# codgodtao/TMDiff

Hardware: AMD Instinct MI355X
Metric: UNet denoise-steps/sec (8-ch 64x64, batch 32) (higher is better)
Workload: dtype f32; 1 GPU; BASELINE configs[1]: batch-32 8-ch 64x64 tiles, DDPM p_sample steps of the T=1000 cosine schedule, channel_multiplier [32,64,128,256], full UNet forward (both branches) + fused DDPM update per step; batch_per_gpu=32, parallelism=batch-parallel x1, weights=key-hashed random init, text_embedding=fixed synthetic 768-d

## Files before the change

include/tmdiff_hip.h:

```cpp
#ifndef TMDIFF_HIP_H
#define TMDIFF_HIP_H

#include <stddef.h>
#include <stdint.h>

#ifdef __cplusplus
extern "C" {
#endif

#define TMDIFF_ABI_VERSION 6

#define TMDIFF_OK 0
#define TMDIFF_E_INVALID (-1)
#define TMDIFF_E_UNSUPPORTED (-2)
#define TMDIFF_E_LAUNCH (-3)

typedef void* tmdiff_stream_t;

int tmdiff_version(void);
const char* tmdiff_last_error_string(void);

typedef struct tmdiff_conv3d_desc {
  int32_t B, N, H, W;
  int32_t Cin, Cout;
// ... 71 lines not shown
int tmdiff_conv3d_wino_pack_weights(const float* w, float* packed, int32_t Cout, int32_t Cin, int32_t groups,
                                    int32_t mode, int32_t planes, tmdiff_stream_t stream);
typedef struct tmdiff_wino_pack_entry {
  const float* w;
  float* packed;
  int32_t Cout, Cin, groups, mode, planes, reserved;
} tmdiff_wino_pack_entry;
int32_t tmdiff_conv3d_wino_pack_weights_multi_chunk(void);
int tmdiff_conv3d_wino_pack_weights_multi(const tmdiff_wino_pack_entry* entries_dev, const int32_t* chunk_tensor_dev,
                                          const int32_t* chunk_index_dev, int32_t n_chunks, tmdiff_stream_t stream);
int tmdiff_conv3d_wino_fwd(const tmdiff_conv3d_desc* d, void* workspace, tmdiff_stream_t stream);
int tmdiff_conv3d_wino_fwd_stage(const tmdiff_conv3d_desc* d, void* workspace, int32_t stage, tmdiff_stream_t stream);
int tmdiff_conv3d_wino_fwd_xp(const tmdiff_conv3d_desc* d, void* workspace, int32_t stage, float* xp_out, tmdiff_stream_t stream);
int tmdiff_conv3d_wino_fwd_planes(const tmdiff_conv3d_desc* d, void* workspace, int32_t stage, float* xp_out, int32_t planes,
                                  tmdiff_stream_t stream);

int tmdiff_conv3d_wf_supported(const tmdiff_conv3d_desc* d);
int64_t tmdiff_conv3d_wf_blocks(const tmdiff_conv3d_desc* d);
size_t tmdiff_conv3d_wf_splitk_workspace_bytes(const tmdiff_conv3d_desc* d);
size_t tmdiff_conv3d_wf_workspace_bytes(const tmdiff_conv3d_desc* d);
int32_t tmdiff_conv3d_wf_plan(int32_t B, int32_t Cin, int32_t Cout, int32_t N, int32_t H, int32_t W, int32_t groups, int32_t llm,
                              int64_t* tiles);
int tmdiff_conv3d_wf_fwd(const tmdiff_conv3d_desc* d, void* workspace, tmdiff_stream_t stream);
int tmdiff_conv3d_wfll_supported(const tmdiff_conv3d_desc* d);
size_t tmdiff_conv3d_wfll_packed_bytes(int32_t Cout, int32_t Cin);
int tmdiff_conv3d_wfll_pack_weights(const float* w, float* packed, int32_t Cout, int32_t Cin, float ll_scale,
                                    tmdiff_stream_t stream);
size_t tmdiff_conv3d_wfll_splitk_workspace_bytes(const tmdiff_conv3d_desc* d);
int tmdiff_conv3d_wfll_fwd(const tmdiff_conv3d_desc* d, float ll_scale, tmdiff_stream_t stream);

size_t tmdiff_conv3d_packed_bf16_bytes(int32_t Cout, int32_t Cin, int32_t ksize, int32_t groups);
int tmdiff_conv3d_pack_weights_bf16(const float* w, void* packed, int32_t Cout, int32_t Cin, int32_t ksize,
                                    int32_t groups, tmdiff_stream_t stream);
int tmdiff_conv3d_pack_weights_bf16_dgrad(const float* w, void* packed, int32_t Cout, int32_t Cin, int32_t ksize,
                                          int32_t groups, tmdiff_stream_t stream);
size_t tmdiff_conv3d_bf16_workspace_bytes(const tmdiff_conv3d_desc* d);
int tmdiff_conv3d_fwd_bf16(const tmdiff_conv3d_desc* d, void* workspace, tmdiff_stream_t stream);


int tmdiff_conv3d_prologue_fwd(const tmdiff_conv3d_desc* d, float* xp, tmdiff_stream_t stream);

size_t tmdiff_conv3d_wgrad_workspace_bytes(const tmdiff_conv3d_desc* d);
int tmdiff_conv3d_wgrad(const tmdiff_conv3d_desc* d, const float* g, float* dw, void* workspace,
                        tmdiff_stream_t stream);
int tmdiff_conv3d_wgrad_bias(const tmdiff_conv3d_desc* d, const float* g, float* dw, float* dbias, void* workspace,
                             tmdiff_stream_t stream);
// ... 261 lines not shown
```

tmdiff_amd/_lib.py:

```python
import ctypes as C
import os

_HERE = os.path.dirname(os.path.abspath(__file__))
LIB_PATH = os.environ.get("TMDIFF_HIP_LIB") or os.path.join(_HERE, "libtmdiff_hip.so")

c_float_p = C.POINTER(C.c_float)
vp = C.c_void_p


class Conv3dDesc(C.Structure):
    _fields_ = [
        ("B", C.c_int32), ("N", C.c_int32), ("H", C.c_int32), ("W", C.c_int32),
        ("Cin", C.c_int32), ("Cout", C.c_int32),
        ("groups", C.c_int32), ("ksize", C.c_int32), ("nseg", C.c_int32),
        ("seg_c", C.c_int32 * 3),
        ("seg_x", vp * 3),
        ("w_packed", vp), ("bias", vp), ("bias_scale", C.c_float),
        ("in_shift", vp), ("in_scale", vp), ("in_shift_stride", C.c_int32), ("in_scale_stride", C.c_int32),
        ("in_mask", vp), ("in_act", C.c_int32),
        ("residual", vp), ("out_scale", C.c_float),
        ("y", vp),
        ("y2", vp), ("y2_shift", vp), ("y2_scale", vp), ("y2_shift_stride", C.c_int32), ("y2_scale_stride", C.c_int32),
        ("y2_act", C.c_int32), ("y2_bf16", C.c_int32), ("x_bf16", C.c_int32),
        ("splitk_ws", vp), ("splitk_ws_bytes", C.c_int64),
# ... 25 lines not shown
    "tmdiff_conv3d_wf_supported": (C.c_int, [C.POINTER(Conv3dDesc)]),
    "tmdiff_conv3d_wf_blocks": (C.c_int64, [C.POINTER(Conv3dDesc)]),
    "tmdiff_conv3d_wf_workspace_bytes": (C.c_size_t, [C.POINTER(Conv3dDesc)]),
    "tmdiff_conv3d_wf_splitk_workspace_bytes": (C.c_size_t, [C.POINTER(Conv3dDesc)]),
    "tmdiff_conv3d_wf_fwd": (C.c_int, [C.POINTER(Conv3dDesc), vp, vp]),
    "tmdiff_conv3d_wino_fwd": (C.c_int, [C.POINTER(Conv3dDesc), vp, vp]),
    "tmdiff_conv3d_wino_fwd_planes": (C.c_int, [C.POINTER(Conv3dDesc), vp, C.c_int32, vp, C.c_int32, vp]),
    "tmdiff_conv3d_wino_fwd_xp": (C.c_int, [C.POINTER(Conv3dDesc), vp, C.c_int32, vp, vp]),
    "tmdiff_conv3d_wino_fwd_stage": (C.c_int, [C.POINTER(Conv3dDesc), vp, C.c_int32, vp]),
    "tmdiff_conv3d_prologue_fwd": (C.c_int, [C.POINTER(Conv3dDesc), vp, vp]),
    "tmdiff_conv3d_ll_supported": (C.c_int, [C.POINTER(Conv3dDesc)]),
    "tmdiff_conv3d_ll_splitk_workspace_bytes": (C.c_size_t, [C.POINTER(Conv3dDesc)]),
    "tmdiff_conv3d_ll_packed_bytes": (C.c_size_t, [C.c_int32, C.c_int32]),
    "tmdiff_conv3d_ll_pack_weights": (C.c_int, [vp, vp, C.c_int32, C.c_int32, C.c_float, vp]),
    "tmdiff_conv3d_ll_fwd": (C.c_int, [C.POINTER(Conv3dDesc), C.c_float, vp]),
    "tmdiff_conv3d_packed_bf16_bytes": (C.c_size_t, [C.c_int32, C.c_int32, C.c_int32, C.c_int32]),
    "tmdiff_conv3d_pack_weights_bf16": (C.c_int, [vp, vp, C.c_int32, C.c_int32, C.c_int32, C.c_int32, vp]),
    "tmdiff_conv3d_bf16_workspace_bytes": (C.c_size_t, [C.POINTER(Conv3dDesc)]),
    "tmdiff_conv3d_fwd_bf16": (C.c_int, [C.POINTER(Conv3dDesc), vp, vp]),
    "tmdiff_conv3d_wgrad_workspace_bytes": (C.c_size_t, [C.POINTER(Conv3dDesc)]),
    "tmdiff_conv3d_wgrad": (C.c_int, [C.POINTER(Conv3dDesc), vp, vp, vp, vp]),
    "tmdiff_conv3d_wgrad_bias": (C.c_int, [C.POINTER(Conv3dDesc), vp, vp, vp, vp, vp]),
    "tmdiff_conv3d_wf_plan": (C.c_int32, [C.c_int32] * 8 + [C.POINTER(C.c_int64)]),
    "tmdiff_conv3d_wfll_supported": (C.c_int, [C.POINTER(Conv3dDesc)]),
    "tmdiff_conv3d_wfll_packed_bytes": (C.c_size_t, [C.c_int32, C.c_int32]),
    "tmdiff_conv3d_wfll_pack_weights": (C.c_int, [vp, vp, C.c_int32, C.c_int32, C.c_float, vp]),
    "tmdiff_conv3d_wfll_splitk_workspace_bytes": (C.c_size_t, [C.POINTER(Conv3dDesc)]),
    "tmdiff_conv3d_wfll_fwd": (C.c_int, [C.POINTER(Conv3dDesc), C.c_float, vp]),
    "tmdiff_conv3d_wgrad_wino_supported": (C.c_int, [C.POINTER(Conv3dDesc)]),
    "tmdiff_conv3d_wgrad_wino_workspace_bytes": (C.c_size_t, [C.POINTER(Conv3dDesc)]),
    "tmdiff_conv3d_wgrad_wino": (C.c_int, [C.POINTER(Conv3dDesc), vp, vp, vp, vp]),
    "tmdiff_conv3d_wgrad_wino_bias": (C.c_int, [C.POINTER(Conv3dDesc), vp, vp, vp, vp, vp]),
    "tmdiff_conv3d_pack_weights_bf16_dgrad": (C.c_int, [vp, vp, C.c_int32, C.c_int32, C.c_int32, C.c_int32, vp]),
    "tmdiff_conv3d_wgrad_bf16_supported": (C.c_int, [C.POINTER(Conv3dDesc)]),
    "tmdiff_conv3d_wgrad_bf16_workspace_bytes": (C.c_size_t, [C.POINTER(Conv3dDesc)]),
    "tmdiff_conv3d_wgrad_bf16_slots": (C.c_int32, [C.POINTER(Conv3dDesc)]),
    "tmdiff_conv3d_wgrad_bf16": (C.c_int, [C.POINTER(Conv3dDesc), vp, vp, vp, vp, vp]),
    "tmdiff_channel_sum": (C.c_int, [vp, vp, C.c_int32, C.c_int32, C.c_int64, C.c_float, vp]),
    "tmdiff_conv3d_prologue_bwd": (C.c_int, [C.POINTER(Conv3dDesc), vp, vp * 3, C.c_int32 * 3, vp, vp, vp]),
    "tmdiff_conv3d_prologue_bwd_workspace_bytes": (C.c_size_t, [C.POINTER(Conv3dDesc)]),
    "tmdiff_conv3d_prologue_bwd_ws": (C.c_int, [C.POINTER(Conv3dDesc), vp, vp * 3, C.c_int32 * 3, vp, vp, vp, vp]),
    "tmdiff_conv3d_prologue_bwd_add": (C.c_int, [C.POINTER(Conv3dDesc), vp, vp * 3, vp * 3, vp, vp, vp, vp]),
    "tmdiff_stem_bwd": (C.c_int, [vp, vp, vp, vp, vp, vp, vp, C.c_int32, C.c_int32, C.c_int32, C.c_int32, C.c_int32, vp]),
    "tmdiff_stem_bwd_input": (C.c_int, [vp, vp, vp, vp, vp, vp, vp, vp, C.c_int32, C.c_int32, C.c_int32, C.c_int32, C.c_int32,
                                        vp]),
    "tmdiff_head_bwd": (C.c_int, [vp, vp, vp, vp, vp, vp, C.c_int32, C.c_int32, C.c_int64, vp]),
# ... 146 lines not shown
```

tmdiff_amd/csrc/conv3d_wf.hip:

```cpp
#include <type_traits>

#include "common.h"
#include "epilogue.h"

#ifndef TMDIFF_WF_ABLATE
#define TMDIFF_WF_ABLATE 0
#endif
#ifndef TMDIFF_WF_STAMPS
#define TMDIFF_WF_STAMPS 0
#endif

namespace {

using namespace tmdiff;

using f32x4 = __attribute__((ext_vector_type(4))) float;
using f32x2 = __attribute__((ext_vector_type(2))) float;

struct WfArgs {
  int B, N, H, W;
  int Cin, Cout, cin_g, cout_g, groups;
  const float* x;
  const float* xgrp[3];
  int grouped_segs;
// ... 21 lines not shown
  const float* rc_x;
  const float* rc_w;
  int rc_cin;
};

#if defined(__HIP_DEVICE_COMPILE__)
using KArgs = const WfArgs __attribute__((address_space(4)))*;
__device__ __forceinline__ KArgs kargs() {
  KArgs k = (KArgs)__builtin_amdgcn_kernarg_segment_ptr();
  asm volatile("" : "+s"(k));
  return k;
}
#else
using KArgs = const WfArgs*;
__device__ __forceinline__ KArgs kargs() { return nullptr; }
#endif

template <class T>
__device__ __forceinline__ T opaque(T v) {
  asm volatile("" : "+v"(v));
  return v;
}

template <int TT, int TH, int TW, bool PAIR = false, bool LLM = false>
struct GeoF {
  static constexpr int NP = 6, MO = 4, NB = TT * MO, KC = 2, CO = 32, NS = 2;
  static constexpr int HH = TH + 2;
  static constexpr int RW = PAIR ? TW : TW + 8, RQ = RW / 4;
  static constexpr int PW = PAIR ? TW + 4 : TW + 2;
  static constexpr int REG_QUADS = NB * RQ;
  static constexpr int PLANES = PAIR ? 32 : 48;
  static constexpr int RPP = PLANES / REG_QUADS;
  static constexpr int NREG = KC * HH;
  static constexpr int XP = (NREG + RPP - 1) / RPP;
  static constexpr int XK = (XP + 3) / 4;
  static constexpr int PSTRIDE = PLANES * 4 + 4;
  static constexpr int RAW_FLOATS = XP * PSTRIDE;
  static constexpr bool SPLIT = TT == 2;
  static constexpr int TSTRIDE = SPLIT ? ((NP * HH * PW + 15) / 32) * 32 + 16 : NP * HH * PW;
  static constexpr int V_ELEMS = (TT - 1) * TSTRIDE + NP * HH * PW;
  static_assert(!SPLIT || (TSTRIDE % 32 == 16 && TSTRIDE >= NP * HH * PW), "tile stride");
  static constexpr int V_FLOATS = KC * V_ELEMS;
  static constexpr int W_TAPS = (LLM ? 4 : 9) * NP;
  static constexpr int W_FLOATS = KC * W_TAPS * CO;
  static constexpr int W_UNITS = W_FLOATS / 4;
  static constexpr int WP = (W_UNITS + 63) / 64, WK = (WP + 3) / 4;
  static constexpr int STAGE = V_FLOATS + WP * 256;
  static constexpr int TCOLS = PAIR ? TW : PW;
  static_assert(REG_QUADS * RPP == PLANES, "a piece holds whole regions");
  static_assert(RPP * TT == 2, "a piece holds two (region, band tile) pairs");
  static_assert(TT * TH * TW == 4 * NS * 32, "4 waves x NS sub-tiles x 32 positions");
  static_assert(TW == 16, "a sub-tile is two rows of 16 positions");
  static_assert(!PAIR || (TT == 2 && TH == 8), "pair mode: two band tiles of 8 rows");
  static_assert(V_FLOATS % 4 == 0, "stage alignment");
};

template <bool Y, bool RES, bool Y2, int TT, int TH, int TW, bool PAIR>
__device__ __forceinline__ void epilogue_wf(KArgs a, f32x16 (&out)[8], float bias_l, float sh2_l, float sc2_l, int b, int g,
                                            int co0, int h0, int w0, int wv, int lane, long plane, float* T, float* ydst,
                                            float oscale, float sh2_m = 0.f, float sc2_m = 1.f, bool pimg_ok = true) {
#pragma clang fp contract(off)
  constexpr int MO = 4, DEPTH = 3;
  const int l31 = lane & 31, khalf = lane >> 5, tq = lane & 7, tc = lane >> 3;
  const int hw = a->H * a->W;
  const long cb = ((long)b * a->Cout + g * a->cout_g + co0) * plane;
  const unsigned span = (unsigned)(((PAIR && pimg_ok ? (long)a->Cout * plane : 0) + 32 * plane) * 4);
  const buf::rsrc ry = buf::make(ydst ? ydst + cb : nullptr, ydst ? span : 0);
  const buf::rsrc rr = buf::make(a->residual ? a->residual + cb : nullptr, a->residual ? span : 0);
  const buf::rsrc r2 = buf::make(a->y2 ? a->y2 + cb : nullptr, a->y2 ? span : 0);
  unsigned toff[2], s2off[2];
// ... 93 lines not shown
        }
      }
      if constexpr (Y2) if (a->y2) {
        float u[4];
#pragma unroll
        for (int e = 0; e < 4; ++e) {
          const float x = v[e] + sh2_t[j];
          const float xa = tmdiff::silu_f(x);
          u[e] = (a->y2_act ? xa : x) * sc2_t[j];
        }
        if (a->y2_s2d) {
          const unsigned o2 = buf::at(s2off[s], (unsigned)((8 * j * (int)plane + n * (hw >> 2)) * 4));
          buf::store2(r2, o2, make_float2(u[0], u[2]));
          buf::store2(r2, buf::at(o2, qplane4), make_float2(u[1], u[3]));
        } else {
          buf::store4(r2, buf::at(toff[s], cj), make_float4(u[0], u[1], u[2], u[3]));
        }
      }
    }
    __builtin_amdgcn_fence(__ATOMIC_SEQ_CST, "wavefront");
  });
}

template <int TT, int TH, int TW, bool PAIR, bool LLM>
__global__ void __launch_bounds__(256, 2) conv3d_wf_kernel(const WfArgs a) {
  using G = GeoF<TT, TH, TW, PAIR, LLM>;
  constexpr int NP = G::NP, MO = G::MO, KC = G::KC, CO = G::CO, NS = G::NS, HH = G::HH, RQ = G::RQ, PW = G::PW;
  constexpr int W_TAPS = G::W_TAPS;
  __shared__ __attribute__((aligned(16))) float lds[2 * G::STAGE + G::RAW_FLOATS];
  float* const st0 = lds;
  float* const st1 = lds + G::STAGE;
  float* const raw = lds + 2 * G::STAGE;
  static_assert(2 * G::STAGE + G::RAW_FLOATS >= 4 * 1024, "the epilogue borrows 4 KB of LDS per wave");

  const int tid = threadIdx.x;
  const int lane = tid & 63, wv = __builtin_amdgcn_readfirstlane(tid >> 6);
  const int l31 = lane & 31, khalf = lane >> 5;
#if TMDIFF_WF_STAMPS
  unsigned long long stamp_t[6];
  const unsigned long long stamp_c0 = __builtin_amdgcn_s_memtime();
  stamp_t[0] = __builtin_amdgcn_s_memrealtime();
#define WF_STAMP(i) stamp_t[i] = __builtin_amdgcn_s_memrealtime()
#else
#define WF_STAMP(i)
#endif
  stagger_start(a.stagger, a.first_round);
  WF_STAMP(1);

  unsigned id = xcd_remap(blockIdx.x, a.total_blocks);
  const int split = take(id, a.ksplit);
  const int co_tile = take(id, a.tiles_co);
  const int tw_i = take(id, a.tiles_w);
  const int th_i = take(id, a.tiles_h);
  const int g = __builtin_amdgcn_readfirstlane(id % a.groups);
  const int b = __builtin_amdgcn_readfirstlane(id / a.groups) * (PAIR ? 2 : 1);
  const bool pimg_ok = !PAIR || b + 1 < a.B;
  const int h0 = th_i * TH, w0 = tw_i * TW;
  const int co0 = co_tile * CO;
  const int hw = a.H * a.W;
  const long plane = (long)a.N * hw;
  const int nchunks = a.split_chunks;
  const float* xg = (a.grouped_segs ? (g == 0 ? a.xgrp[0] : (g == 1 ? a.xgrp[1] : a.xgrp[2])) + (long)b * a.cin_g * plane
                                    : a.x + ((long)b * a.Cin + (long)g * a.cin_g) * plane) + (long)split * nchunks * KC * plane;
  const float* wg = a.wp + ((long)g * a.cin_g + (long)split * nchunks * KC) * W_TAPS * a.cout_g + co0;

  const long xbs = PAIR && pimg_ok ? (long)(a.grouped_segs ? a.cin_g : a.Cin) * plane : 0;
  const unsigned xbytes = (unsigned)((xbs + KC * plane) * 4), wbytes = (unsigned)(KC * W_TAPS * a.cout_g * 4);
  const int xq = lane % G::REG_QUADS, xsub = lane / G::REG_QUADS;
  unsigned xlane_off;
  if constexpr (PAIR) {
    const int img = (xq % RQ) >> 1;
    xlane_off = (lane < G::PLANES && (img == 0 || pimg_ok)) ? (unsigned)((img * xbs + (xq / RQ) * hw + 4 * (xq & 1)) * 4) : buf::kOutside;
  } else {
    const int xwq = w0 - 4 + 4 * (xq % RQ);
    xlane_off = (lane < G::PLANES && xwq >= 0 && xwq < a.W) ? (unsigned)(((xq / RQ) * hw + xwq) * 4) : buf::kOutside;
  }
  auto issue_raw = [&](auto kc_, int c) __attribute__((always_inline)) {
    constexpr int k = decltype(kc_)::value;
    const int p = wv + 4 * k;
    if (G::XP % 4 == 0 || p < G::XP) {
      const buf::rsrc r = buf::make(xg + (long)c * KC * plane, xbytes);
      const int region = p * G::RPP + (G::RPP > 1 ? xsub : 0);
      const int kc = region / HH, row = region - kc * HH;
      const int h = h0 - 1 + row;
      const bool ok = h >= 0 && h < a.H && region < G::NREG;
      const unsigned lo = opaque(xlane_off);
      const unsigned voff = ok ? lo + (unsigned)((kc * (int)plane + h * a.W) * 4) : buf::kOutside;
      if (lane < G::PLANES) buf::dma_b128(r, lo >= buf::kOutside ? buf::kOutside : voff, 0, raw + p * G::PSTRIDE);
    }
  };
  const unsigned wlane_off = (unsigned)(((lane >> 3) * a.cout_g + (lane & 7) * 4) * 4);
  auto issue_w = [&](auto kc_, int c, float* st) __attribute__((always_inline)) {
    constexpr int k = decltype(kc_)::value;
    const int q = wv + 4 * k;
    if (G::WP % 4 == 0 || q < G::WP) {
      const buf::rsrc r = buf::make(wg + (long)c * KC * W_TAPS * a.cout_g, wbytes);
      buf::dma_b128(r, opaque(wlane_off) + (unsigned)(q * 8 * a.cout_g * 4), 0, st + G::V_FLOATS + q * 256);
    }
  };

  constexpr int TC = G::TCOLS;
  constexpr int TPP = G::RPP * TT * TC;
  constexpr int NTASK = G::XK * TPP, NTR = (NTASK + 63) / 64;
  int trd[NTR], twr[NTR];
  bool tlo[NTR], thi[NTR];
#pragma unroll
  for (int j = 0; j < NTR; ++j) {
    int id = j * 64 + lane;
    if (id >= NTASK) id -= TPP;
    if (wv + 4 * (id / TPP) >= G::XP) id -= TPP;
    const int tpi = id / TPP, rem = id % TPP, sub = rem / TC, col = rem % TC;
    const int tp = wv + 4 * tpi;
    const int ttile = G::RPP == 1 ? sub : 0, trsub = G::RPP == 1 ? 0 : sub;
    const int tregion = tp * G::RPP + trsub;
    const int tkc = tregion / HH, trow = tregion - tkc * HH;
    trd[j] = tp * G::PSTRIDE + trsub * (G::REG_QUADS * 4) + (MO * ttile) * (RQ * 4) + col + (PAIR ? 0 : 3);
    twr[j] = tkc * G::V_ELEMS + ttile * G::TSTRIDE + trow * PW + (PAIR ? col + 1 + 2 * (col >> 3) : col);
    tlo[j] = ttile > 0, thi[j] = ttile < TT - 1;
  }
  float tin[NP];
  auto tr_load = [&](auto jc) __attribute__((always_inline)) {
    constexpr int j = decltype(jc)::value;
    const float* src = raw + opaque(trd[j]);
#pragma unroll
    for (int i = 0; i < NP; ++i) tin[i] = src[(i - 1) * (RQ * 4)];
  };
  auto tr_col = [&](auto jc, float* st) __attribute__((always_inline)) {
    constexpr int j = decltype(jc)::value;
    const float d0 = tlo[j] ? tin[0] : 0.f, d1 = tin[1], d2 = tin[2], d3 = tin[3], d4 = tin[4], d5 = thi[j] ? tin[5] : 0.f;
    const float a42 = d4 - 4.f * d2, b31 = d3 - 4.f * d1, c42 = d4 - d2, e31 = d3 - d1;
    float* dst = st + opaque(twr[j]);
    dst[0 * HH * PW] = (4.f * d0 + d4) - 5.f * d2;
    dst[1 * HH * PW] = a42 + b31;
    dst[2 * HH * PW] = a42 - b31;
    dst[3 * HH * PW] = c42 + 2.f * e31;
    dst[4 * HH * PW] = c42 - 2.f * e31;
    dst[5 * HH * PW] = (4.f * d1 + d5) - 5.f * d3;
  };

  constexpr int SUB_STEP = G::SPLIT ? PW : 2 * PW;
  const int boff = khalf * G::V_ELEMS + (G::SPLIT ? (l31 >> 4) * G::TSTRIDE + (2 * wv) * PW + (l31 & 15) + (PAIR ? 2 * ((l31 & 15) >> 3) : 0)
                                                  : (4 * wv + (l31 >> 4)) * PW + (l31 & 15)) + (LLM ? 1 - khalf : 0);
  const int aoff = G::V_FLOATS + khalf * W_TAPS * CO + l31;

  float bias_l, sh2_l, sc2_l, sh2_m = 0.f, sc2_m = 1.f;
  {
    const int col = g * a.cout_g + co0 + l31;
    bias_l = a.bias ? a.bias[col] * a.bias_scale : 0.f;
    const bool has2 = a.y2 || a.yhi[0];
    sh2_l = (has2 && a.y2_shift) ? a.y2_shift[(long)b * a.y2_shift_stride + col] : 0.f;
    sc2_l = (has2 && a.y2_scale) ? a.y2_scale[(long)b * a.y2_scale_stride + col] : 1.f;
    if constexpr (PAIR) {
      const int b1 = pimg_ok ? b + 1 : b;
      sh2_m = (a.y2 && a.y2_shift) ? a.y2_shift[(long)b1 * a.y2_shift_stride + col] : 0.f;
      sc2_m = (a.y2 && a.y2_scale) ? a.y2_scale[(long)b1 * a.y2_scale_stride + col] : 1.f;
    }
  }
  if constexpr (PAIR) {
    constexpr int ROWS = G::V_FLOATS / PW;
    static_assert(ROWS * PW == G::V_FLOATS, "the planes of a stage are one run of rows");
    for (int i = tid; i < 2 * ROWS * 4; i += 256) {
      const int stg = i / (ROWS * 4), r = (i >> 2) % ROWS, q = i & 3;
      lds[stg * G::STAGE + r * PW + (q == 0 ? 0 : (q == 1 ? 9 : (q == 2 ? 10 : 19)))] = 0.f;
    }
  }

  f32x16 acc[NP * NS];
#pragma unroll
  for (int i = 0; i < NP * NS; ++i)
#pragma unroll
    for (int r = 0; r < 16; ++r) acc[i][r] = 0.f;

  static_for<0, G::XK>([&](auto k) __attribute__((always_inline)) { issue_raw(k, 0); });
  static_for<0, G::WK>([&](auto k) __attribute__((always_inline)) { issue_w(k, 0, st0); });
  __builtin_amdgcn_s_waitcnt(0x0F70);
  static_for<0, NTR>([&](auto jc) __attribute__((always_inline)) { tr_load(jc); tr_col(jc, st0); });
  static_for<0, G::XK>([&](auto k) __attribute__((always_inline)) { issue_raw(k, nchunks > 1 ? 1 : 0); });
  __syncthreads();
  WF_STAMP(2);

  constexpr int KSTEPS = W_TAPS;
  constexpr int SLOT_COL0 = 0, COL_STEP = LLM ? 4 : 6, SLOT_W0 = LLM ? 12 : 20, SLOT_RAW0 = LLM ? 14 : 26, STEP = LLM ? 1 : 2;
  static_assert(SLOT_COL0 + NTR * COL_STEP <= SLOT_W0 + 1 && SLOT_W0 + G::WK <= SLOT_RAW0 && SLOT_RAW0 + G::XK * STEP <= KSTEPS - (LLM ? 4 : 8),
                "work items in order, raw pieces early enough to land");
// ... 47 lines not shown
      __syncthreads();
    }
  }
  WF_STAMP(3);

#pragma unroll
  for (int s = 0; s < NS; ++s)
#pragma unroll
    for (int r = 0; r < 16; ++r) {
      const float m0 = acc[0 * NS + s][r], m1 = acc[1 * NS + s][r], m2 = acc[2 * NS + s][r], m3 = acc[3 * NS + s][r],
                  m4 = acc[4 * NS + s][r], m5 = acc[5 * NS + s][r];
      const float p12 = m1 + m2, d12 = m1 - m2, p34 = m3 + m4, d34 = m3 - m4;
      acc[0 * NS + s][r] = (m0 + p12) + p34;
      acc[1 * NS + s][r] = d12 + 2.f * d34;
      acc[2 * NS + s][r] = p12 + 4.f * p34;
      acc[3 * NS + s][r] = (d12 + 8.f * d34) + m5;
    }
  f32x16 out[8];
#pragma unroll
  for (int i = 0; i < 8; ++i) out[i] = acc[(i % MO) * NS + i / MO];
  if constexpr (!PAIR && !LLM) {
    if (a.rc_x && split == 0) {
      __syncthreads();
      float* wl = lds;
      for (int e = tid; e < a.rc_cin * 32; e += 256) {
        const int co = e / a.rc_cin, ci = e - co * a.rc_cin;
        wl[ci * 32 + co] = a.rc_w[(long)(co0 + co) * a.rc_cin + ci];
      }
      __syncthreads();
      const buf::rsrc xr = buf::make(a.rc_x + (long)b * a.rc_cin * plane, (unsigned)((long)a.rc_cin * plane * 4));
      unsigned xo[8];
#pragma unroll
      for (int i = 0; i < 8; ++i) {
        const int s_ = i / MO, n_ = i % MO;
        const int bt = TT == 2 ? l31 >> 4 : 0;
        const int h = h0 + (TT == 2 ? 2 * wv + s_ : 4 * wv + 2 * s_ + (l31 >> 4)), w = w0 + (l31 & 15);
        xo[i] = (unsigned)((khalf * (int)plane + ((h < a.H && w < a.W) ? (MO * bt + n_) * hw + h * a.W + w : 0)) * 4);
      }
      constexpr int GJ = 16;
      const int ngrp = a.rc_cin / (2 * GJ);
      const unsigned pair_bytes = (unsigned)(2 * plane * 4);
      float xv[2][GJ];
      auto fetch = [&](int jg, auto ic, auto slotc) __attribute__((always_inline)) {
        constexpr int i = decltype(ic)::value, slot = decltype(slotc)::value;
        const unsigned s0 = (unsigned)(jg * GJ) * pair_bytes;
#pragma unroll
        for (int j = 0; j < GJ; ++j) xv[slot][j] = buf::load(xr, xo[i], s0 + (unsigned)j * pair_bytes);
      };
      fetch(0, std::integral_constant<int, 0>{}, std::integral_constant<int, 0>{});
      for (int jg = 0; jg < ngrp; ++jg) {
        const float* wrow = wl + (jg * 2 * GJ + khalf) * 32 + l31;
        static_for<0, 8>([&](auto ic) __attribute__((always_inline)) {
          constexpr int i = decltype(ic)::value, slot = i & 1;
          if constexpr (i < 7) fetch(jg, std::integral_constant<int, i + 1>{}, std::integral_constant<int, slot ^ 1>{});
          else if (jg + 1 < ngrp) fetch(jg + 1, std::integral_constant<int, 0>{}, std::integral_constant<int, 0>{});
#pragma unroll
          for (int j = 0; j < GJ; ++j) out[i] = __builtin_amdgcn_mfma_f32_32x32x2f32(wrow[2 * j * 32], xv[slot][j], out[i], 0, 0, 0);
        });
      }
      __syncthreads();
    }
  }
  float* T = lds + wv * 1024;
  const KArgs ea = kargs();
#define WF_EPI2(Y, R, Y2) \
  epilogue_wf<Y, R, Y2, TT, TH, TW, PAIR>(ea, out, bias_l, sh2_l, sc2_l, b, g, co0, h0, w0, wv, lane, plane, T, a.y, a.out_scale, sh2_m, sc2_m, pimg_ok)
  if (a.part) {
    float* pd = a.part + (long)split * a.B * a.Cout * plane;
    epilogue_wf<true, false, false, TT, TH, TW, PAIR>(ea, out, 0.f, 0.f, 1.f, b, g, co0, h0, w0, wv, lane, plane, T, pd, 1.f, 0.f, 1.f, pimg_ok);
  } else if (a.y) {
    if (a.residual) { if (a.y2) WF_EPI2(true, true, true); else WF_EPI2(true, true, false); }
    else            { if (a.y2) WF_EPI2(true, false, true); else WF_EPI2(true, false, false); }
  } else {
    if (a.residual) WF_EPI2(false, true, true); else WF_EPI2(false, false, true);
  }
#undef WF_EPI2
#if TMDIFF_WF_STAMPS
  WF_STAMP(4);
  __builtin_amdgcn_s_waitcnt(0);
  WF_STAMP(5);
  if (a.stamps && lane == 0) {
    unsigned long long* o = a.stamps + ((unsigned long long)blockIdx.x * 4 + wv) * 8;
    for (int i = 0; i < 6; ++i) o[i] = stamp_t[i];
    o[6] = ((unsigned long long)__builtin_amdgcn_s_getreg(4 | (31 << 11)) << 32) | __builtin_amdgcn_s_getreg(6 | (31 << 11)) |
           ((unsigned long long)(__builtin_amdgcn_s_getreg(20 | (31 << 11)) & 0xf) << 28);
    o[7] = __builtin_amdgcn_s_memtime() - stamp_c0;
  }
#endif
}

template <int TT, int TH, int TW, bool PAIR = false, bool LLM = false>
int launch(WfArgs& a, hipStream_t st) {
  a.tiles_h = (a.H + TH - 1) / TH;
  a.tiles_w = PAIR ? 1 : (a.W + TW - 1) / TW;
  a.tiles_co = a.cout_g / 32;
  const long blocks = (long)a.ksplit * (PAIR ? (a.B + 1) / 2 : a.B) * a.groups * a.tiles_h * a.tiles_w * a.tiles_co;
  if (const int rc = tmdiff::set_grid(a, blocks, "conv3d_wf_fwd")) return rc;
  static const double stagger_chunks = env_double("TMDIFF_WF_STAGGER", 0.0);
  a.first_round = 512;
  a.stagger = blocks > 512 ? (int)(stagger_chunks * 2.0 * 54 * 2 * 64) : 0;
  conv3d_wf_kernel<TT, TH, TW, PAIR, LLM><<<(unsigned)blocks, 256, 0, st>>>(a);
  return tmdiff::check_launch("conv3d_wf_fwd");
}

bool wf_form_ok(const tmdiff_conv3d_desc* d) {
  if (!d || d->ksize != 3 || (d->groups != 1 && d->groups != 3) || d->in_mask || d->x_bf16 || d->y2_bf16) return false;
  if (!(d->drop_p >= 0.f && d->drop_p < 1.f)) return false;
  if (d->nseg < 1 || d->nseg > 3 || d->Cin <= 0 || d->Cout <= 0 || d->Cin % d->groups || d->Cout % d->groups) return false;
  return (d->Cin / d->groups) % 2 == 0 && (d->Cout / d->groups) % 32 == 0 && (d->N == 8 || d->N == 4) && d->H > 0 && d->W > 0 &&
         d->W % 4 == 0;
}

bool wf_grouped_segs(const tmdiff_conv3d_desc* d) {
  return d->nseg == 3 && d->groups == 3 && d->seg_c[0] == d->seg_c[1] && d->seg_c[1] == d->seg_c[2] &&
         d->seg_c[0] * 3 == d->Cin;
}

bool wf_pair(const tmdiff_conv3d_desc* d) { return d->N == 8 && d->W == 8; }

bool wf_plain(const tmdiff_conv3d_desc* d) {
  return (d->nseg == 1 || wf_grouped_segs(d)) && !d->in_shift && !d->in_scale && !d->in_act && !(d->drop_p > 0.f);
}

bool wf_fits(const tmdiff_conv3d_desc* d) {
// ... 11 lines not shown
  const long units = wf_pair(d) ? (d->B + 1) / 2 : (long)d->B * ((d->W + 15) / 16);
  return units * d->groups * ((d->H + th - 1) / th) * (d->Cout / d->groups / 32);
}

int wf_ksplit(const tmdiff_conv3d_desc* d, bool pairs = false) {
  static const long target = env_long("TMDIFF_SPLITK", 256);
  const long tiles = wf_tiles(d);
  const int nchunks = d->Cin / d->groups / 2;
  const int ksteps = pairs ? 24 : 54;
  if (target <= 0 || tiles <= 0) return 1;
  auto ok = [&](int s) { return s >= 1 && nchunks % s == 0 && nchunks / s >= 2 && !(pairs && (nchunks / s) % 2); };
  int best = 1;
  if (tiles < target)
    for (int s = 2; s <= nchunks / 2; ++s) {
      if (!ok(s)) continue;
      best = s;
      if (tiles * s >= target) break;
    }
  static const long long_range = env_long("TMDIFF_SPLITK_LONG", 1700);
  if (tiles * best < 384 && ok(2 * best) && (long)(nchunks / (2 * best)) * ksteps >= long_range) best *= 2;
  return best;
}

}

extern "C" int tmdiff_conv3d_wf_supported(const tmdiff_conv3d_desc* d) { return wf_shape_ok(d) ? 1 : 0; }

extern "C" int32_t tmdiff_conv3d_wf_plan(int32_t B, int32_t Cin, int32_t Cout, int32_t N, int32_t H, int32_t W, int32_t groups,
                                         int32_t llm, int64_t* tiles) {
  tmdiff_conv3d_desc d = {};
  d.B = B; d.N = N; d.H = H; d.W = W; d.Cin = Cin; d.Cout = Cout; d.groups = groups; d.ksize = 3; d.nseg = 1; d.seg_c[0] = Cin;
  if (tiles) *tiles = 0;
  if (B <= 0 || !wf_shape_ok(&d)) return 0;
  if (tiles) *tiles = wf_tiles(&d);
  return wf_ksplit(&d, llm != 0);
}

extern "C" int64_t tmdiff_conv3d_wf_blocks(const tmdiff_conv3d_desc* d) {
  if (!wf_shape_ok(d) || d->B <= 0) return 0;
  return (int64_t)wf_tiles(d) * wf_ksplit(d);
}

extern "C" size_t tmdiff_conv3d_wf_splitk_workspace_bytes(const tmdiff_conv3d_desc* d) {
  if (!wf_shape_ok(d) || d->B <= 0) return 0;
  return splitk_bytes(wf_ksplit(d), d, (long)d->N * d->H * d->W);
}
// ... 49 lines not shown
    }
  }
  a.yll = nullptr; a.yhi[0] = a.yhi[1] = a.yhi[2] = nullptr;
  if (d->y_ll) {
    const bool dwt = d->y_hi[0] != nullptr;
    if (llm || wf_pair(d) || a.part || d->y || (dwt ? (d->y2 || !d->y_hi[1] || !d->y_hi[2]) : !d->y2) || d->N != 8 || d->H % 2 ||
        d->W % 4 || !aligned16(d->y_ll) || !aligned16(d->y_hi[0]) || !aligned16(d->y_hi[1]) || !aligned16(d->y_hi[2]))
      return fail(TMDIFF_E_UNSUPPORTED, "conv3d_wf_fwd: the LL / Haar output needs 8 bands, even H, W %% 4 == 0, planes wider than 8 columns, "
                                        "y == NULL (with a second output, or with all three high bands and none), and a grid that "
                                        "does not split its input channels");
    a.yll = d->y_ll;
    for (int i = 0; i < 3; ++i) a.yhi[i] = dwt ? d->y_hi[i] : nullptr;
  }
  a.rc_x = nullptr; a.rc_w = nullptr; a.rc_cin = 0;
  if (d->rc_x) {
    if (llm || wf_pair(d) || d->groups != 1 || d->residual || !d->rc_w || d->rc_cin <= 0 || d->rc_cin % 32 || d->rc_cin > 512 ||
        !aligned16(d->rc_x) || !aligned16(d->rc_w))
      return fail(TMDIFF_E_UNSUPPORTED, "conv3d_wf_fwd: a folded residual convolution needs groups 1, rc_cin %% 32 == 0 (at most 512), no residual "
                                        "tensor and planes wider than 8 columns");
    if (!wf_rc_fits(d)) return fail(TMDIFF_E_UNSUPPORTED, "conv3d_wf_fwd: rc_x sample too large for 32-bit byte offsets");
    a.rc_x = d->rc_x; a.rc_w = d->rc_w; a.rc_cin = d->rc_cin;
  }
  int rc;
  if (llm) rc = wf_pair(d) ? launch<2, 8, 16, true, true>(a, st) : (d->N == 8 ? launch<2, 8, 16, false, true>(a, st) : launch<1, 16, 16, false, true>(a, st));
  else rc = wf_pair(d) ? launch<2, 8, 16, true>(a, st) : (d->N == 8 ? launch<2, 8, 16>(a, st) : launch<1, 16, 16>(a, st));
  if (rc || !a.part) return rc;
  return finish_splitk(a, d, plane, d->bias_scale, st);
}

bool wfll_desc(const tmdiff_conv3d_desc* d, tmdiff_conv3d_desc* e) {
  if (!d || d->ksize != 3 || d->groups != 1 || d->nseg != 1 || (d->N != 8 && d->N != 4) || d->H <= 0 || d->W <= 0 || d->H % 2 || d->W % 8) return false;
  if (d->in_shift || d->in_scale || d->in_act || d->in_mask || d->drop_p > 0.f || d->x_bf16 || d->y2_bf16 || d->y2_s2d) return false;
  if (d->Cin <= 0 || d->Cout <= 0 || d->Cout % 32 || d->seg_c[0] != d->Cin) return false;
  *e = *d;
  e->H = d->H / 2; e->W = d->W / 2; e->Cin = 4 * d->Cin; e->seg_c[0] = 4 * d->Cin;
  return wf_shape_ok(e);
}

__constant__ float kG6[6][3] = {{0.25f, 0.f, 0.f},           {-1.f / 6.f, -1.f / 6.f, -1.f / 6.f}, {-1.f / 6.f, 1.f / 6.f, -1.f / 6.f},
                                {1.f / 24.f, 1.f / 12.f, 1.f / 6.f}, {1.f / 24.f, -1.f / 12.f, 1.f / 6.f}, {0.f, 0.f, 1.f}};

__global__ void __launch_bounds__(256) wfll_pack_kernel(const float* __restrict__ w, float* __restrict__ packed, int Cout, int Cin, float s) {
  const long r = blockIdx.x * 256L + threadIdx.x;
  if (r >= (long)Cout * Cin) return;
  const int co = (int)(r % Cout), ci = (int)(r / Cout);
  const float* wk = w + ((long)co * Cin + ci) * 27;
  float t[27];
#pragma unroll
// ... 69 lines not shown
```

tmdiff_amd/ops.py:

```python
import ctypes as C
import math
import os

import numpy as np
import torch

from . import _lib, routing
from ._lib import Conv3dDesc, check, lib



class KernelConfig:

    _FLAG = lambda default: (lambda v: (v != "0") if default else (v == "1"))
    _FIELDS = {
        "winograd": ("TMDIFF_WINOGRAD", _FLAG(True), True), "wf": ("TMDIFF_WF", _FLAG(True), True),
        "wf_pair": ("TMDIFF_WF_PAIR", _FLAG(True), True), "wf_splitk": ("TMDIFF_WF_SPLITK", _FLAG(True), True),
        "wf_min_fill": ("TMDIFF_WF_MIN_FILL", float, 0.7), "wino_min_blocks": ("TMDIFF_WINO_MIN_BLOCKS", int, 256),
        "ll_compose": ("TMDIFF_LL_COMPOSE", _FLAG(True), True), "wfll": ("TMDIFF_WFLL", _FLAG(True), True),
        "train_ll_wino": ("TMDIFF_TRAIN_LL_WINO", _FLAG(True), True),
        "conv2_after_ll": ("TMDIFF_CONV2_AFTER_LL", _FLAG(True), True),
        "epilogue_fuse": ("TMDIFF_EPILOGUE_FUSE", _FLAG(True), True), "producer_fuse": ("TMDIFF_PRODUCER_FUSE", _FLAG(True), True),
        "fp32_staged": ("TMDIFF_FP32_STAGED", str, "auto"), "bf16_pack": ("TMDIFF_BF16_PACK", str, "auto"),
        "wgrad_wino": ("TMDIFF_WGRAD_WINO", _FLAG(True), True), "wgrad_wino_bias": ("TMDIFF_WGRAD_WINO_BIAS", _FLAG(True), True),
# ... 598 lines not shown
        if not routing.wf_quarter_ok(b, cin, cout, n, h, w, groups):
            raise ValueError("conv3d_wf: this launch cannot write a space-to-depth / LL output (ask routing.wf_quarter_ok first)")
    if want_ll and keep_y:
        raise ValueError("conv3d_wf: the LL output replaces y (keep_y=False)")
    q = (b, cout, n, h // 2, w // 2)
    y_ll = torch.empty(*q, device=dev, dtype=torch.float32) if want_ll else None
    y_hi = [torch.empty(*q, device=dev, dtype=torch.float32) for _ in range(3)] if want_dwt else None
    y, y2 = _outputs("conv3d_wf", dev, (b, cout, n, h, w), keep_y, emit,
                     None if want_dwt else ((b, 4 * cout, n, h // 2, w // 2) if s2d else (b, cout, n, h, w)))
    d = make_conv_desc(segs, w_packed, cout, 3, y, y2=y2, groups=groups, y2_s2d=s2d, y_ll=y_ll, y_hi=y_hi, **kw,
                       **_emit_kw(emit))
    if not lib.tmdiff_conv3d_wf_supported(C.byref(d)):
        raise ValueError("conv3d_wf: shape not supported")
    _lend_splitk(d, dev, lib.tmdiff_conv3d_wf_splitk_workspace_bytes(C.byref(d)) if (config.wf_splitk and not want_ll) else 0)
    nws = lib.tmdiff_conv3d_wf_workspace_bytes(C.byref(d))
    ws = _xp_target("conv3d_wf", xp_out, nws, dev)
    if xp_out is not None and not nws:
        xp_out.copy_(segs[0] if len(segs) == 1 else torch.cat(segs, 1))
    flops = 2.0 * b * cout * ((d.Cin // groups) * 13.5 + d.rc_cin) * n * h * w
    _launch(lib.tmdiff_conv3d_wf_fwd, d, (ws,), "conv3d_wf_fwd", "conv3d_wf_fwd", flops, 3, f" +rc{d.rc_cin}" if d.rc_cin else "")
    return (y_ll, *y_hi) if want_dwt else (y2, y_ll) if want_ll else _result(y, y2)


def pack_conv_weight_ll(w, ll_scale=0.5):
    cout, cin = w.shape[0], w.shape[1]
    nb = lib.tmdiff_conv3d_ll_packed_bytes(cout, cin)
    if tuple(w.shape[2:]) != (3, 3, 3) or nb == 0:
        raise ValueError(f"pack_conv_weight_ll: weight shape {tuple(w.shape)} not supported")
    out = torch.empty(nb // 4, device=w.device, dtype=torch.float32)
    check(lib.tmdiff_conv3d_ll_pack_weights(_chk(w.detach(), "w"), out.data_ptr(), cout, cin, float(ll_scale), stream_ptr()),
          "conv3d_ll_pack_weights")
    return out


def conv3d_ll(x, w_packed, cout, ll_scale=0.5, emit=None, keep_y=True, **kw):
    b, _, n, h, w = x.shape
    dev = x.device
    oshape = (b, cout, n, h // 2, w // 2)
    y, y2 = _outputs("conv3d_ll", dev, oshape, keep_y, emit, oshape)
    d = make_conv_desc([x], w_packed, cout, 3, y, y2=y2, out_div=2, **kw, **_emit_kw(emit))
    if not lib.tmdiff_conv3d_ll_supported(C.byref(d)):
        raise ValueError("conv3d_ll: shape not supported (ll_conv_supported)")
    _lend_splitk(d, dev, lib.tmdiff_conv3d_ll_splitk_workspace_bytes(C.byref(d)))
    _launch(lib.tmdiff_conv3d_ll_fwd, d, (float(ll_scale),), "conv3d_ll_fwd", "conv3d_ll_fwd",
            2.0 * b * cout * d.Cin * 48 * n * (h // 2) * (w // 2))
    return _result(y, y2)
# ... 1118 lines not shown
```

Before: 45.17 batch32-steps/s.

## Let one workgroup compute two 32-channel output tiles in the wf Winograd conv

```diff
diff --git a/include/tmdiff_hip.h b/include/tmdiff_hip.h
--- a/include/tmdiff_hip.h
+++ b/include/tmdiff_hip.h
@@ -117,6 +117,9 @@
 int32_t tmdiff_conv3d_wf_plan(int32_t B, int32_t Cin, int32_t Cout, int32_t N, int32_t H, int32_t W, int32_t groups, int32_t llm,
                               int64_t* tiles);
 int tmdiff_conv3d_wf_fwd(const tmdiff_conv3d_desc* d, void* workspace, tmdiff_stream_t stream);
+void tmdiff_conv3d_wf_set_cw(int32_t cw);
+int32_t tmdiff_conv3d_wf_cw(int32_t B, int32_t Cin, int32_t Cout, int32_t N, int32_t H, int32_t W, int32_t groups, int32_t llm,
+                            int32_t rc_cin);
 int tmdiff_conv3d_wfll_supported(const tmdiff_conv3d_desc* d);
 size_t tmdiff_conv3d_wfll_packed_bytes(int32_t Cout, int32_t Cin);
 int tmdiff_conv3d_wfll_pack_weights(const float* w, float* packed, int32_t Cout, int32_t Cin, float ll_scale,
diff --git a/tmdiff_amd/_lib.py b/tmdiff_amd/_lib.py
--- a/tmdiff_amd/_lib.py
+++ b/tmdiff_amd/_lib.py
@@ -71,6 +71,8 @@
     "tmdiff_conv3d_wgrad": (C.c_int, [C.POINTER(Conv3dDesc), vp, vp, vp, vp]),
     "tmdiff_conv3d_wgrad_bias": (C.c_int, [C.POINTER(Conv3dDesc), vp, vp, vp, vp, vp]),
     "tmdiff_conv3d_wf_plan": (C.c_int32, [C.c_int32] * 8 + [C.POINTER(C.c_int64)]),
+    "tmdiff_conv3d_wf_set_cw": (None, [C.c_int32]),
+    "tmdiff_conv3d_wf_cw": (C.c_int32, [C.c_int32] * 9),
     "tmdiff_conv3d_wfll_supported": (C.c_int, [C.POINTER(Conv3dDesc)]),
     "tmdiff_conv3d_wfll_packed_bytes": (C.c_size_t, [C.c_int32, C.c_int32]),
     "tmdiff_conv3d_wfll_pack_weights": (C.c_int, [vp, vp, C.c_int32, C.c_int32, C.c_float, vp]),
diff --git a/tmdiff_amd/csrc/conv3d_wf.hip b/tmdiff_amd/csrc/conv3d_wf.hip
--- a/tmdiff_amd/csrc/conv3d_wf.hip
+++ b/tmdiff_amd/csrc/conv3d_wf.hip
@@ -1,3 +1,4 @@
+#include <atomic>
 #include <type_traits>
 
 #include "common.h"
@@ -67,8 +68,12 @@
   return v;
 }
 
-template <int TT, int TH, int TW, bool PAIR = false, bool LLM = false>
+constexpr int kRcCinMax[2] = {512, 384};
+
+template <int TT, int TH, int TW, bool PAIR = false, bool LLM = false, int CW = 1>
 struct GeoF {
+  static_assert(CW == 1 || CW == 2, "one or two 32-channel tiles per workgroup");
+  static constexpr int NW = 4 * CW, NT = 64 * NW;
   static constexpr int NP = 6, MO = 4, NB = TT * MO, KC = 2, CO = 32, NS = 2;
   static constexpr int HH = TH + 2;
   static constexpr int RW = PAIR ? TW : TW + 8, RQ = RW / 4;
@@ -78,7 +83,7 @@
   static constexpr int RPP = PLANES / REG_QUADS;
   static constexpr int NREG = KC * HH;
   static constexpr int XP = (NREG + RPP - 1) / RPP;
-  static constexpr int XK = (XP + 3) / 4;
+  static constexpr int XK = (XP + NW - 1) / NW;
   static constexpr int PSTRIDE = PLANES * 4 + 4;
   static constexpr int RAW_FLOATS = XP * PSTRIDE;
   static constexpr bool SPLIT = TT == 2;
@@ -89,8 +94,10 @@
   static constexpr int W_TAPS = (LLM ? 4 : 9) * NP;
   static constexpr int W_FLOATS = KC * W_TAPS * CO;
   static constexpr int W_UNITS = W_FLOATS / 4;
-  static constexpr int WP = (W_UNITS + 63) / 64, WK = (WP + 3) / 4;
-  static constexpr int STAGE = V_FLOATS + WP * 256;
+  static constexpr int WP = (W_UNITS + 63) / 64;
+  static constexpr int WPT = CW * WP, WK = (WPT + NW - 1) / NW;
+  static constexpr int STAGE = V_FLOATS + WPT * 256;
+  static constexpr int LDS_FLOATS = 2 * STAGE + RAW_FLOATS;
   static constexpr int TCOLS = PAIR ? TW : PW;
   static_assert(REG_QUADS * RPP == PLANES, "a piece holds whole regions");
   static_assert(RPP * TT == 2, "a piece holds two (region, band tile) pairs");
@@ -230,19 +237,22 @@
   });
 }
 
-template <int TT, int TH, int TW, bool PAIR, bool LLM>
-__global__ void __launch_bounds__(256, 2) conv3d_wf_kernel(const WfArgs a) {
-  using G = GeoF<TT, TH, TW, PAIR, LLM>;
+template <int TT, int TH, int TW, bool PAIR, bool LLM, int CW>
+__global__ void __launch_bounds__(256 * CW, 2 / CW) conv3d_wf_kernel(const WfArgs a) {
+  using G = GeoF<TT, TH, TW, PAIR, LLM, CW>;
+  constexpr int NW = G::NW;
   constexpr int NP = G::NP, MO = G::MO, KC = G::KC, CO = G::CO, NS = G::NS, HH = G::HH, RQ = G::RQ, PW = G::PW;
   constexpr int W_TAPS = G::W_TAPS;
-  __shared__ __attribute__((aligned(16))) float lds[2 * G::STAGE + G::RAW_FLOATS];
+  __shared__ __attribute__((aligned(16))) float lds[G::LDS_FLOATS];
   float* const st0 = lds;
   float* const st1 = lds + G::STAGE;
   float* const raw = lds + 2 * G::STAGE;
-  static_assert(2 * G::STAGE + G::RAW_FLOATS >= 4 * 1024, "the epilogue borrows 4 KB of LDS per wave");
+  static_assert(G::LDS_FLOATS >= NW * 1024, "the epilogue borrows 4 KB of LDS per wave");
+  static_assert(PAIR || LLM || G::LDS_FLOATS >= kRcCinMax[CW - 1] * 32 * CW, "the folded residual convolution's weight slabs lie in the stages");
 
   const int tid = threadIdx.x;
-  const int lane = tid & 63, wv = __builtin_amdgcn_readfirstlane(tid >> 6);
+  const int lane = tid & 63, wq = __builtin_amdgcn_readfirstlane(tid >> 6);
+  const int wv = CW == 2 ? wq & 3 : wq, ct = CW == 2 ? wq >> 2 : 0;
   const int l31 = lane & 31, khalf = lane >> 5;
 #if TMDIFF_WF_STAMPS
   unsigned long long stamp_t[6];
@@ -264,13 +274,13 @@
   const int b = __builtin_amdgcn_readfirstlane(id / a.groups) * (PAIR ? 2 : 1);
   const bool pimg_ok = !PAIR || b + 1 < a.B;
   const int h0 = th_i * TH, w0 = tw_i * TW;
-  const int co0 = co_tile * CO;
+  const int co0 = (co_tile * CW + ct) * CO;
   const int hw = a.H * a.W;
   const long plane = (long)a.N * hw;
   const int nchunks = a.split_chunks;
   const float* xg = (a.grouped_segs ? (g == 0 ? a.xgrp[0] : (g == 1 ? a.xgrp[1] : a.xgrp[2])) + (long)b * a.cin_g * plane
                                     : a.x + ((long)b * a.Cin + (long)g * a.cin_g) * plane) + (long)split * nchunks * KC * plane;
-  const float* wg = a.wp + ((long)g * a.cin_g + (long)split * nchunks * KC) * W_TAPS * a.cout_g + co0;
+  const float* wg = a.wp + ((long)g * a.cin_g + (long)split * nchunks * KC) * W_TAPS * a.cout_g + co_tile * (CW * CO);
 
   const long xbs = PAIR && pimg_ok ? (long)(a.grouped_segs ? a.cin_g : a.Cin) * plane : 0;
   const unsigned xbytes = (unsigned)((xbs + KC * plane) * 4), wbytes = (unsigned)(KC * W_TAPS * a.cout_g * 4);
@@ -285,8 +295,8 @@
   }
   auto issue_raw = [&](auto kc_, int c) __attribute__((always_inline)) {
     constexpr int k = decltype(kc_)::value;
-    const int p = wv + 4 * k;
-    if (G::XP % 4 == 0 || p < G::XP) {
+    const int p = wq + NW * k;
+    if (G::XP % NW == 0 || p < G::XP) {
       const buf::rsrc r = buf::make(xg + (long)c * KC * plane, xbytes);
       const int region = p * G::RPP + (G::RPP > 1 ? xsub : 0);
       const int kc = region / HH, row = region - kc * HH;
@@ -300,10 +310,15 @@
   const unsigned wlane_off = (unsigned)(((lane >> 3) * a.cout_g + (lane & 7) * 4) * 4);
   auto issue_w = [&](auto kc_, int c, float* st) __attribute__((always_inline)) {
     constexpr int k = decltype(kc_)::value;
-    const int q = wv + 4 * k;
-    if (G::WP % 4 == 0 || q < G::WP) {
+    const int q = wq + NW * k;
+    if (G::WPT % NW == 0 || q < G::WPT) {
       const buf::rsrc r = buf::make(wg + (long)c * KC * W_TAPS * a.cout_g, wbytes);
-      buf::dma_b128(r, opaque(wlane_off) + (unsigned)(q * 8 * a.cout_g * 4), 0, st + G::V_FLOATS + q * 256);
+      if constexpr (CW == 1) {
+        buf::dma_b128(r, opaque(wlane_off) + (unsigned)(q * 8 * a.cout_g * 4), 0, st + G::V_FLOATS + q * 256);
+      } else {
+        const int t = q >= G::WP ? 1 : 0, qr = q - t * G::WP;
+        buf::dma_b128(r, opaque(wlane_off) + (unsigned)((qr * 8 * a.cout_g + t * CO) * 4), 0, st + G::V_FLOATS + q * 256);
+      }
     }
   };
 
@@ -316,9 +331,9 @@
   for (int j = 0; j < NTR; ++j) {
     int id = j * 64 + lane;
     if (id >= NTASK) id -= TPP;
-    if (wv + 4 * (id / TPP) >= G::XP) id -= TPP;
+    if (wq + NW * (id / TPP) >= G::XP) id -= TPP;
     const int tpi = id / TPP, rem = id % TPP, sub = rem / TC, col = rem % TC;
-    const int tp = wv + 4 * tpi;
+    const int tp = wq + NW * tpi;
     const int ttile = G::RPP == 1 ? sub : 0, trsub = G::RPP == 1 ? 0 : sub;
     const int tregion = tp * G::RPP + trsub;
     const int tkc = tregion / HH, trow = tregion - tkc * HH;
@@ -349,7 +364,7 @@
   constexpr int SUB_STEP = G::SPLIT ? PW : 2 * PW;
   const int boff = khalf * G::V_ELEMS + (G::SPLIT ? (l31 >> 4) * G::TSTRIDE + (2 * wv) * PW + (l31 & 15) + (PAIR ? 2 * ((l31 & 15) >> 3) : 0)
                                                   : (4 * wv + (l31 >> 4)) * PW + (l31 & 15)) + (LLM ? 1 - khalf : 0);
-  const int aoff = G::V_FLOATS + khalf * W_TAPS * CO + l31;
+  const int aoff = G::V_FLOATS + ct * (G::WP * 256) + khalf * W_TAPS * CO + l31;
 
   float bias_l, sh2_l, sc2_l, sh2_m = 0.f, sc2_m = 1.f;
   {
@@ -367,7 +382,7 @@
   if constexpr (PAIR) {
     constexpr int ROWS = G::V_FLOATS / PW;
     static_assert(ROWS * PW == G::V_FLOATS, "the planes of a stage are one run of rows");
-    for (int i = tid; i < 2 * ROWS * 4; i += 256) {
+    for (int i = tid; i < 2 * ROWS * 4; i += G::NT) {
       const int stg = i / (ROWS * 4), r = (i >> 2) % ROWS, q = i & 3;
       lds[stg * G::STAGE + r * PW + (q == 0 ? 0 : (q == 1 ? 9 : (q == 2 ? 10 : 19)))] = 0.f;
     }
@@ -461,10 +476,11 @@
   if constexpr (!PAIR && !LLM) {
     if (a.rc_x && split == 0) {
       __syncthreads();
-      float* wl = lds;
-      for (int e = tid; e < a.rc_cin * 32; e += 256) {
+      float* wl = lds + ct * (a.rc_cin * 32);
+      for (int e = tid; e < a.rc_cin * (32 * CW); e += G::NT) {
         const int co = e / a.rc_cin, ci = e - co * a.rc_cin;
-        wl[ci * 32 + co] = a.rc_w[(long)(co0 + co) * a.rc_cin + ci];
+        if constexpr (CW == 1) wl[ci * 32 + co] = a.rc_w[(long)(co0 + co) * a.rc_cin + ci];
+        else lds[(co >> 5) * (a.rc_cin * 32) + ci * 32 + (co & 31)] = a.rc_w[(long)(co_tile * (CW * CO) + co) * a.rc_cin + ci];
       }
       __syncthreads();
       const buf::rsrc xr = buf::make(a.rc_x + (long)b * a.rc_cin * plane, (unsigned)((long)a.rc_cin * plane * 4));
@@ -500,7 +516,7 @@
       __syncthreads();
     }
   }
-  float* T = lds + wv * 1024;
+  float* T = lds + wq * 1024;
   const KArgs ea = kargs();
 #define WF_EPI2(Y, R, Y2) \
   epilogue_wf<Y, R, Y2, TT, TH, TW, PAIR>(ea, out, bias_l, sh2_l, sc2_l, b, g, co0, h0, w0, wv, lane, plane, T, a.y, a.out_scale, sh2_m, sc2_m, pimg_ok)
@@ -519,7 +535,7 @@
   __builtin_amdgcn_s_waitcnt(0);
   WF_STAMP(5);
   if (a.stamps && lane == 0) {
-    unsigned long long* o = a.stamps + ((unsigned long long)blockIdx.x * 4 + wv) * 8;
+    unsigned long long* o = a.stamps + ((unsigned long long)blockIdx.x * NW + wq) * 8;
     for (int i = 0; i < 6; ++i) o[i] = stamp_t[i];
     o[6] = ((unsigned long long)__builtin_amdgcn_s_getreg(4 | (31 << 11)) << 32) | __builtin_amdgcn_s_getreg(6 | (31 << 11)) |
            ((unsigned long long)(__builtin_amdgcn_s_getreg(20 | (31 << 11)) & 0xf) << 28);
@@ -529,16 +545,17 @@
 }
 
 template <int TT, int TH, int TW, bool PAIR = false, bool LLM = false>
-int launch(WfArgs& a, hipStream_t st) {
+int launch(WfArgs& a, int cw, hipStream_t st) {
   a.tiles_h = (a.H + TH - 1) / TH;
   a.tiles_w = PAIR ? 1 : (a.W + TW - 1) / TW;
-  a.tiles_co = a.cout_g / 32;
+  a.tiles_co = a.cout_g / (32 * cw);
   const long blocks = (long)a.ksplit * (PAIR ? (a.B + 1) / 2 : a.B) * a.groups * a.tiles_h * a.tiles_w * a.tiles_co;
   if (const int rc = tmdiff::set_grid(a, blocks, "conv3d_wf_fwd")) return rc;
   static const double stagger_chunks = env_double("TMDIFF_WF_STAGGER", 0.0);
   a.first_round = 512;
   a.stagger = blocks > 512 ? (int)(stagger_chunks * 2.0 * 54 * 2 * 64) : 0;
-  conv3d_wf_kernel<TT, TH, TW, PAIR, LLM><<<(unsigned)blocks, 256, 0, st>>>(a);
+  if (cw == 2) conv3d_wf_kernel<TT, TH, TW, PAIR, LLM, 2><<<(unsigned)blocks, 512, 0, st>>>(a);
+  else conv3d_wf_kernel<TT, TH, TW, PAIR, LLM, 1><<<(unsigned)blocks, 256, 0, st>>>(a);
   return tmdiff::check_launch("conv3d_wf_fwd");
 }
 
@@ -596,6 +613,39 @@
   return best;
 }
 
+std::atomic<int> g_wf_cw{0};
+constexpr long kCwMinBlocks32 = 512;
+constexpr int kCwPlainMinChunks = 32;
+constexpr int kCwPlainMinCoutG = 128;
+constexpr int kCwPairMinChunks = 48;
+constexpr bool kCwLl = true;
+
+bool wf_cw2_legal(const tmdiff_conv3d_desc* d) {
+  return (d->Cout / d->groups) % 64 == 0 && (!d->rc_x || d->rc_cin <= kRcCinMax[1]);
+}
+
+int wf_cw(const tmdiff_conv3d_desc* d, int ksplit, bool llm) {
+  const int forced = g_wf_cw.load(std::memory_order_relaxed);
+  if (forced == 1 || !wf_cw2_legal(d)) return 1;
+  if (forced == 2) return 2;
+  if (wf_tiles(d) * ksplit < kCwMinBlocks32) return 1;
+  const int chunks = d->Cin / d->groups / 2 / ksplit;
+  if (llm) return kCwLl ? 2 : 1;
+  if (wf_pair(d)) return chunks >= kCwPairMinChunks ? 2 : 1;
+  return chunks >= kCwPlainMinChunks && d->Cout / d->groups >= kCwPlainMinCoutG ? 2 : 1;
+}
+
+}
+
+extern "C" void tmdiff_conv3d_wf_set_cw(int32_t cw) { g_wf_cw.store(cw == 1 || cw == 2 ? cw : 0, std::memory_order_relaxed); }
+
+extern "C" int32_t tmdiff_conv3d_wf_cw(int32_t B, int32_t Cin, int32_t Cout, int32_t N, int32_t H, int32_t W, int32_t groups, int32_t llm,
+                                       int32_t rc_cin) {
+  tmdiff_conv3d_desc d = {};
+  d.B = B; d.N = N; d.H = H; d.W = W; d.Cin = Cin; d.Cout = Cout; d.groups = groups; d.ksize = 3; d.nseg = 1; d.seg_c[0] = Cin;
+  if (B <= 0 || !wf_shape_ok(&d)) return 0;
+  if (rc_cin > 0) { d.rc_x = reinterpret_cast<const float*>(&d); d.rc_cin = rc_cin; }
+  return wf_cw(&d, wf_ksplit(&d, llm != 0), llm != 0);
 }
 
 extern "C" int tmdiff_conv3d_wf_supported(const tmdiff_conv3d_desc* d) { return wf_shape_ok(d) ? 1 : 0; }
@@ -691,8 +741,9 @@
     a.rc_x = d->rc_x; a.rc_w = d->rc_w; a.rc_cin = d->rc_cin;
   }
   int rc;
-  if (llm) rc = wf_pair(d) ? launch<2, 8, 16, true, true>(a, st) : (d->N == 8 ? launch<2, 8, 16, false, true>(a, st) : launch<1, 16, 16, false, true>(a, st));
-  else rc = wf_pair(d) ? launch<2, 8, 16, true>(a, st) : (d->N == 8 ? launch<2, 8, 16>(a, st) : launch<1, 16, 16>(a, st));
+  const int cw = wf_cw(d, a.ksplit, llm);
+  if (llm) rc = wf_pair(d) ? launch<2, 8, 16, true, true>(a, cw, st) : (d->N == 8 ? launch<2, 8, 16, false, true>(a, cw, st) : launch<1, 16, 16, false, true>(a, cw, st));
+  else rc = wf_pair(d) ? launch<2, 8, 16, true>(a, cw, st) : (d->N == 8 ? launch<2, 8, 16>(a, cw, st) : launch<1, 16, 16>(a, cw, st));
   if (rc || !a.part) return rc;
   return finish_splitk(a, d, plane, d->bias_scale, st);
 }
diff --git a/tmdiff_amd/ops.py b/tmdiff_amd/ops.py
--- a/tmdiff_amd/ops.py
+++ b/tmdiff_amd/ops.py
@@ -644,6 +644,14 @@
     return (y_ll, *y_hi) if want_dwt else (y2, y_ll) if want_ll else _result(y, y2)
 
 
+def wf_set_cw(cw=0):
+    lib.tmdiff_conv3d_wf_set_cw(int(cw))
+
+
+def wf_cw(b, cin, cout, n, h, w, groups=1, llm=False, rc_cin=0):
+    return int(lib.tmdiff_conv3d_wf_cw(b, cin, cout, n, h, w, groups, 1 if llm else 0, rc_cin))
+
+
 def pack_conv_weight_ll(w, ll_scale=0.5):
     cout, cin = w.shape[0], w.shape[1]
     nb = lib.tmdiff_conv3d_ll_packed_bytes(cout, cin)
```

After: 45.56 batch32-steps/s (median of 6 runs). About the same (+0.9%).
